# ml4ai/mliis

Hardware: AMD Instinct MI355X
Metric: inner-loop images/sec (EfficientLab-6-3, 224x224, 5-shot) (higher is better)
Workload: dtype f32 (the long-K decoder convs and their filter gradients with every operand split exactly into three bf16 terms on the matrix cores, 6 term products, f32 accumulate: fp32-equivalent products; everything else the fp32 instruction)

## Files before the change

### mliis_amd/csrc/dwmarch.hip

```cpp
#include "bn_fold.hpp"
#include "common.hpp"

namespace mliis {

constexpr int kDwmStoreAux = 2;
typedef unsigned dwm_u32x4 __attribute__((ext_vector_type(4)));
constexpr unsigned kDwmOob = 0xFFFFFFF0u;

__device__ __forceinline__ __amdgpu_buffer_rsrc_t dwm_rsrc(const void* p) {
  const unsigned long long u = (unsigned long long)p;
  const unsigned lo = __builtin_amdgcn_readfirstlane((unsigned)u), hi = __builtin_amdgcn_readfirstlane((unsigned)(u >> 32));
  return __builtin_amdgcn_make_buffer_rsrc((void*)(((unsigned long long)hi << 32) | lo), 0, 0x80000000u, 0x00020000);
}

typedef unsigned dwm_u32x2 __attribute__((ext_vector_type(2)));
template <typename T = float>
__device__ __forceinline__ float4 dwm_load(__amdgpu_buffer_rsrc_t r, int off, bool ok) {
  if constexpr (sizeof(T) == 4) {
    const dwm_u32x4 u = __builtin_amdgcn_raw_buffer_load_b128(r, ok ? off : (int)kDwmOob, 0, 0);
    return make_float4(__uint_as_float(u.x), __uint_as_float(u.y), __uint_as_float(u.z), __uint_as_float(u.w));
  } else {
    const dwm_u32x2 u = __builtin_amdgcn_raw_buffer_load_b64(r, ok ? off : (int)kDwmOob, 0, 0);
    return unpack_bf16x4(make_uint2(u.x, u.y));
  }
}

template <typename T = float>
__device__ __forceinline__ void dwm_store(__amdgpu_buffer_rsrc_t r, int off, bool ok, const float4 v) {
  if constexpr (sizeof(T) == 2) {
    const uint2 pk = pack_bf16x4(v);
    dwm_u32x2 u2;
    u2.x = pk.x; u2.y = pk.y;
    __builtin_amdgcn_raw_buffer_store_b64(u2, r, ok ? off : (int)kDwmOob, 0, kDwmStoreAux);
    return;
  }
  dwm_u32x4 u;
  u.x = __float_as_uint(v.x); u.y = __float_as_uint(v.y); u.z = __float_as_uint(v.z); u.w = __float_as_uint(v.w);
  __builtin_amdgcn_raw_buffer_store_b128(u, r, ok ? off : (int)kDwmOob, 0, kDwmStoreAux);
}
__device__ __forceinline__ float4 f4sel(bool ok, const float4 v) { return ok ? v : make_float4(0.f, 0.f, 0.f, 0.f); }
template <typename T> __device__ __forceinline__ float4 dwm_stored(const float4 v) { return stored_value(static_cast<const T*>(nullptr), v); }

template <int K, int S>
struct MarchCfg {
  static constexpr int TS = S == 1 ? 4 : 2;
  static constexpr int BW = 7 * TS;
  static constexpr int SPR = BW / TS;
  static constexpr int RS = 4;
  static constexpr int IBW = (BW - 1) * S + K;
  static constexpr int IBWP = (IBW + 1) & ~1;
  static constexpr int WIN = (RS - 1) * S + K;
  static constexpr int NEW = RS * S;
  static constexpr int NR = WIN + NEW;
  static constexpr int WW = (TS - 1) * S + K;
  static_assert(IBW <= 32, "one pixel lane per ring column");
  static_assert(WIN <= 2 * NEW, "head batch + batch 0 cover the window of step 0");
};

struct DwmBn {
  BnFold f;
  const float* gamma;
  const float* beta;
};

struct DwmDyBn {
  const float* z;
  const float *mean, *rstd, *gamma, *beta;
  const float *gate, *chan_add;
  const float* stage1;
  int nimg;
  double inv_rows;
  float *dgamma, *dbeta;
};
struct DwmDyQuad {
  float4 sc, sh, gt, ca, k1, k0;
};
__device__ __forceinline__ DwmDyQuad dwm_dybn_setup(const DwmDyBn& d, int C, int c0, int q, bool cok, int n, bool lead) {
  const int c = cok ? c0 + q * 4 : 0;
  const float4 m = ld4(d.mean + c), rs = ld4(d.rstd + c), ga = ld4(d.gamma + c), be = ld4(d.beta + c);
  DwmDyQuad k;
  k.gt = ld4(d.gate + (long long)n * C + c);
  k.ca = ld4(d.chan_add + (long long)n * C + c);
  double s1[4] = {0, 0, 0, 0}, s2[4] = {0, 0, 0, 0};
  for (int i0 = 0; i0 < d.nimg; i0 += 8) {
    float4 u[8], v[8];
#pragma unroll
    for (int j = 0; j < 8; ++j) {
      const int i = i0 + j < d.nimg ? i0 + j : d.nimg - 1;
      u[j] = ld4(d.stage1 + ((long long)i * 2 + 0) * C + c);
      v[j] = ld4(d.stage1 + ((long long)i * 2 + 1) * C + c);
    }
#pragma unroll
    for (int j = 0; j < 8; ++j)
      if (i0 + j < d.nimg) {
        s1[0] += u[j].x; s1[1] += u[j].y; s1[2] += u[j].z; s1[3] += u[j].w;
        s2[0] += v[j].x; s2[1] += v[j].y; s2[2] += v[j].z; s2[3] += v[j].w;
      }
  }
  if (lead && cok && (threadIdx.x >> 3) == 0) {
    st4(d.dbeta + c, make_float4((float)s1[0], (float)s1[1], (float)s1[2], (float)s1[3]));
    st4(d.dgamma + c, make_float4((float)s2[0], (float)s2[1], (float)s2[2], (float)s2[3]));
  }
  const float4 a = make_float4((float)(s1[0] * d.inv_rows), (float)(s1[1] * d.inv_rows), (float)(s1[2] * d.inv_rows), (float)(s1[3] * d.inv_rows));
  const float4 b = make_float4((float)(s2[0] * d.inv_rows), (float)(s2[1] * d.inv_rows), (float)(s2[2] * d.inv_rows), (float)(s2[3] * d.inv_rows));
  k.sc = f4mul(ga, rs);
  k.sh = make_float4(fmaf(-m.x, k.sc.x, be.x), fmaf(-m.y, k.sc.y, be.y), fmaf(-m.z, k.sc.z, be.z), fmaf(-m.w, k.sc.w, be.w));
  k.k1 = make_float4(-k.sc.x * b.x * rs.x, -k.sc.y * b.y * rs.y, -k.sc.z * b.z * rs.z, -k.sc.w * b.w * rs.w);
  k.k0 = make_float4(-k.sc.x * a.x - k.k1.x * m.x, -k.sc.y * a.y - k.k1.y * m.y, -k.sc.z * a.z - k.k1.z * m.z, -k.sc.w * a.w - k.k1.w * m.w);
  return k;
}
__device__ __forceinline__ float dwm_dz1(float da2, float z, float sc, float sh, float gt, float ca, float k1, float k0) {
  const float u = fmaf(z, sc, sh);
  const float sg = sigmoid_f(u);
  const float g = fmaf(da2, gt, ca) * (sg * (1.0f + u * (1.0f - sg)));
  return fmaf(sc, g, fmaf(z, k1, k0));
}
__device__ __forceinline__ float4 dwm_dz1(const float4 da2, const float4 z, const DwmDyQuad& k) {
  return make_float4(dwm_dz1(da2.x, z.x, k.sc.x, k.sh.x, k.gt.x, k.ca.x, k.k1.x, k.k0.x), dwm_dz1(da2.y, z.y, k.sc.y, k.sh.y, k.gt.y, k.ca.y, k.k1.y, k.k0.y),
                     dwm_dz1(da2.z, z.z, k.sc.z, k.sh.z, k.gt.z, k.ca.z, k.k1.z, k.k0.z), dwm_dz1(da2.w, z.w, k.sc.w, k.sh.w, k.gt.w, k.ca.w, k.k1.w, k.k0.w));
}

template <int NEW, bool TWO>
struct DwmBatch {
  float4 a[NEW];
  float4 b[TWO ? NEW : 1];
};

struct DwmArgs {
  const float* x;
  const float* w;
  float* y;
  int Hi, Wi, Ho, Wo;
  int C, pt, pl;
  int bands, bw, chunks, rpc;
  float* stats_part;
  DwmBn bn;
  DwmDyBn dyb;
  const float* z;
  float* dw_part;
};

struct DwmQuad {
  float4 sc, sh, m, rs;
};

__device__ __forceinline__ float4 dwm_act(const float4 z, const DwmQuad& k) {
  float4 u = make_float4(fmaf(z.x, k.sc.x, k.sh.x), fmaf(z.y, k.sc.y, k.sh.y), fmaf(z.z, k.sc.z, k.sh.z), fmaf(z.w, k.sc.w, k.sh.w));
  return make_float4(swish_f(u.x), swish_f(u.y), swish_f(u.z), swish_f(u.w));
}

constexpr int kDwmFoldBatch = 8;
template <bool FOLD>
struct DwmBnState {
  float4 g, b, m, rs;
  FoldAcc acc;
  float4 u[FOLD ? kDwmFoldBatch : 1], v[FOLD ? kDwmFoldBatch : 1];
  int k;
};
template <bool FOLD>
__device__ __forceinline__ void dwm_bn_begin(const DwmBn& bn, int C, int c0, int q, bool cok, DwmBnState<FOLD>& st) {
  const int c = cok ? c0 + q * 4 : 0;
  st.g = ld4(bn.gamma + c);
  st.b = ld4(bn.beta + c);
  if (FOLD && bn.f.nblk > 0) {
    const int bl = threadIdx.x >> 3;
    st.k = bl;
    for (; st.k + 32 * kDwmFoldBatch < bn.f.nblk; st.k += 32 * kDwmFoldBatch) {
      fold_issue<FOLD ? kDwmFoldBatch : 1>(bn.f.part, bn.f.nblk, C, c, st.k, bl, st.u, st.v);
      if (cok) fold_add<FOLD ? kDwmFoldBatch : 1>(st.acc, bn.f.nblk, st.k, st.u, st.v);
    }
    fold_issue<FOLD ? kDwmFoldBatch : 1>(bn.f.part, bn.f.nblk, C, c, st.k, st.k < bn.f.nblk ? st.k : 0, st.u, st.v);
  } else {
    st.m = ld4(bn.f.mean + c);
    st.rs = ld4(bn.f.rstd + c);
  }
}
template <bool FOLD>
__device__ __forceinline__ DwmQuad dwm_bn_end(const DwmBn& bn, int C, int c0, int q, bool cok, bool lead, double* smd, float* s_mr ,
                                              DwmBnState<FOLD>& st) {
  const int t = threadIdx.x;
  DwmQuad k;
  if (FOLD && bn.f.nblk > 0) {
    if (cok) fold_add<FOLD ? kDwmFoldBatch : 1>(st.acc, bn.f.nblk, st.k, st.u, st.v);
    double s, ss;
    fold_finish(st.acc, smd, s, ss);
    if (t < 32) {
      const double m = s * bn.f.inv_n;
      double var = ss * bn.f.inv_n - m * m;
      if (var < 0.0) var = 0.0;
      const float mf = (float)m, rf = (float)(1.0 / sqrt(var + (double)bn.f.eps));
      s_mr[t] = mf;
      s_mr[32 + t] = rf;
      const int cc = c0 + t;
      if (lead && cc < C) {
        bn.f.mean[cc] = mf;
        bn.f.rstd[cc] = rf;
        if (bn.f.moving_mean != nullptr) {
          const float mm = bn.f.moving_mean[cc], mv = bn.f.moving_var[cc];
          bn.f.moving_mean[cc] = mm - (mm - mf) * bn.f.one_minus_momentum;
          bn.f.moving_var[cc] = mv - (mv - (float)(var * (double)bn.f.ema_var_factor)) * bn.f.one_minus_momentum;
        }
      }
    }
    __syncthreads();
    k.m = ld4(s_mr + q * 4);
    k.rs = ld4(s_mr + 32 + q * 4);
    __syncthreads();
  } else {
    k.m = st.m;
    k.rs = st.rs;
  }
  k.sc = f4mul(st.g, k.rs);
  k.sh = make_float4(fmaf(-k.m.x, k.sc.x, st.b.x), fmaf(-k.m.y, k.sc.y, st.b.y), fmaf(-k.m.z, k.sc.z, st.b.z), fmaf(-k.m.w, k.sc.w, st.b.w));
  return k;
}

__device__ __forceinline__ void dwm_emit_pair(const float4 s1, const float4 s2, float4* buf, float* __restrict__ part, unsigned blk, int C,
                                              int c0) {
  const int t = threadIdx.x;
  buf[t] = s1;
  buf[256 + t] = s2;
  __syncthreads();
  float4 v = f4zero();
  if (t < 64) {
    const int qq = t & 7, g = (t >> 3) & 3, vv = t >> 5;
#pragma unroll
    for (int i = 0; i < 8; ++i) v = f4add(v, buf[vv * 256 + (g * 8 + i) * 8 + qq]);
  }
  __syncthreads();
  if (t < 64) buf[t] = v;
  __syncthreads();
  if (t < 16) {
    const int qq = t & 7, vv = t >> 3;
    const int cc = c0 + qq * 4;
    const float4* b4 = buf + vv * 32 + qq;
    if (cc < C) st4(part + ((long long)blk * 2 + vv) * C + cc, f4add(f4add(b4[0], b4[8]), f4add(b4[16], b4[24])));
  }
}

template <int K, int S, bool PRE, bool BWD, bool DYBN = false, typename TA = float, typename TB = float>
__global__ __launch_bounds__(256, BWD ? 1 : 2) void dwm_conv_k(const DwmArgs a) {
  constexpr int EA = (int)sizeof(TA), EB = (int)sizeof(TB);
  static_assert(!DYBN || BWD, "DYBN is a backward mode");
  typedef MarchCfg<K, S> G;
  constexpr int TS = G::TS, SPR = G::SPR, RS = G::RS, IBW = G::IBW, IBWP = G::IBWP, WIN = G::WIN, NEW = G::NEW, NR = G::NR, WW = G::WW;
  static_assert(!BWD || S == 1, "the stride-2 backward is dwm_bwd_s2_k");
  constexpr int kRingF4 = (NR * IBWP + 1) * 8;
  constexpr int kTrash = NR * IBWP * 8;
  constexpr int kScratchF4 = BWD ? (K * K * 4 * 8) : 0;
  constexpr int kSharedF4 = kRingF4 > kScratchF4 ? kRingF4 : kScratchF4;
  static_assert(kSharedF4 * 16 >= 2 * 32 * 32 * 8, "the statistics fold borrows the ring");
  __shared__ float4 ring[kSharedF4];
  __shared__ float4 wl[K * K * 8];
  __shared__ __attribute__((aligned(16))) float s_mr[64];

  const int t = threadIdx.x, q = t & 7, p = t >> 3;
  const unsigned bx = xcd_remap(blockIdx.x, gridDim.x);
  const int chunk = (int)(bx % (unsigned)a.chunks);
  const unsigned r_ = bx / (unsigned)a.chunks;
  const int band = (int)(r_ % (unsigned)a.bands), n = (int)(r_ / (unsigned)a.bands);
  const int c0 = blockIdx.y * 32, c = c0 + q * 4;
  const bool cok = c < a.C;
  const int Hi = a.Hi, Wi = a.Wi, Ho = a.Ho, Wo = a.Wo, C = a.C;
  const int oy0 = chunk * a.rpc;
  const int oy1 = oy0 + a.rpc < Ho ? oy0 + a.rpc : Ho;
  const int ox0 = band * a.bw;
  const int bwa = a.bw < Wo - ox0 ? a.bw : Wo - ox0;
  const int iy0 = oy0 * S - a.pt, ix0 = ox0 * S - a.pl;
  const int ibw = (bwa - 1) * S + K;
  const int rows_needed = (oy1 - oy0 - 1) * S + K;
  const int nsteps = (oy1 - oy0 + RS - 1) / RS;
  const __amdgpu_buffer_rsrc_t rX = dwm_rsrc(a.x);
  const __amdgpu_buffer_rsrc_t rZ = dwm_rsrc((BWD ? a.z : a.x));
  const __amdgpu_buffer_rsrc_t rY = dwm_rsrc(a.y);

  const bool colok = cok && p < ibw && (unsigned)(ix0 + p) < (unsigned)Wi;
  const int tbase = (((n * Hi + iy0) * Wi + ix0 + p) * C + c) * EA;
  const int rowbytes = Wi * C * EA;
  const int lcol = p < IBWP ? (p ^ ((p >> 2) & 1)) * 8 + q : kTrash + q;
  auto row_in = [&](int rr) { return rr >= 0 && rr < rows_needed && (unsigned)(iy0 + rr) < (unsigned)Hi; };
  typedef DwmBatch<NEW, DYBN> Batch;
  const __amdgpu_buffer_rsrc_t rX2 = dwm_rsrc(DYBN ? a.dyb.z : a.x);
  auto issue = [&](Batch& r, int rb) {
#pragma unroll
    for (int j = 0; j < NEW; ++j) {
      r.a[j] = dwm_load<TA>(rX, tbase + (rb + j) * rowbytes, colok && row_in(rb + j));
      if (DYBN) r.b[j] = dwm_load<TA>(rX2, tbase + (rb + j) * rowbytes, colok && row_in(rb + j));
    }
  };
  DwmQuad kq;
  DwmDyQuad dq;
  auto commit = [&](const Batch& r, int rb, int sb) {
#pragma unroll
    for (int j = 0; j < NEW; ++j) {
      float4 v = r.a[j];
      if (PRE && !BWD) v = f4sel(colok && row_in(rb + j), dwm_act(v, kq));
      if (DYBN) v = f4sel(colok && row_in(rb + j), dwm_dz1(v, r.b[j], dq));
      int slot = sb + j;
      if (slot >= NR) slot -= NR;
      if (rb + j >= 0) ring[(p < IBWP ? slot * (IBWP * 8) : 0) + lcol] = v;
    }
  };

  const int ro = p >> 3, sx = p & 7;
  const bool item_ok = sx < SPR && cok;
  const int colbase = sx < SPR ? sx * (TS * S) : 0;
  const int sxpar = sx & 1;
  const int zbase = BWD ? (((n * Ho + oy0 + ro) * Wo + ox0 + sx * TS) * C + c) * EB : 0;
  auto issue_z = [&](float4 (&zr)[TS], int step) {
    if (BWD) {
      const int oy = oy0 + step * RS + ro;
      const int base = zbase + step * RS * Wo * C * EB;
#pragma unroll
      for (int u = 0; u < TS; ++u) zr[u] = dwm_load<TB>(rZ, base + u * C * EB, item_ok && oy < oy1 && sx * TS + u < bwa);
    }
  };

  constexpr int HEAD = WIN - 2 * NEW;
  float4 wreg = f4zero();
  if (t < K * K * 8) {
    const int tap = t >> 3, qq = t & 7;
    const int cc = c0 + qq * 4;
    if (cc < C) wreg = ld4(a.w + (long long)(BWD ? K * K - 1 - tap : tap) * C + cc);
  }
  DwmBnState<!BWD> bst;
  if (PRE) dwm_bn_begin(a.bn, C, c0, q, cok, bst);
  if (DYBN) dq = dwm_dybn_setup(a.dyb, C, c0, q, cok, n, bx == 0);
  Batch ra, rb_;
  float4 za[TS], zb[TS];
  {
    Batch h0, h1;
    issue(h0, HEAD);
    issue(h1, WIN - NEW);
    issue_z(za, 0);
    if (PRE) kq = dwm_bn_end(a.bn, C, c0, q, cok, bx == 0, reinterpret_cast<double*>(ring), s_mr, bst);
    issue(ra, WIN);
    issue(rb_, WIN + NEW);
    issue_z(zb, 1);
    if (t < K * K * 8) wl[t] = wreg;
    commit(h0, HEAD, HEAD < 0 ? HEAD + NR : HEAD);
    commit(h1, WIN - NEW, (WIN - NEW) % NR);
  }
  __syncthreads();

  float4 s1 = f4zero(), s2 = f4zero();
  float4 dwacc[BWD ? K * K : 1];
  if (BWD) {
#pragma unroll
    for (int k = 0; k < K * K; ++k) dwacc[k] = f4zero();
  }

  int sw = 0;
  auto compute = [&](int step, const float4 (&zr)[TS]) {
    const int oy = oy0 + step * RS + ro;
    const bool row_ok = item_ok && oy < oy1;
    int s0 = sw + ro * S;
    if (s0 >= NR) s0 -= NR;
    float4 acc[TS];
#pragma unroll
    for (int u = 0; u < TS; ++u) acc[u] = f4zero();
    int wofs = q;
    if (K == 5) asm volatile("" : "+v"(wofs));
    const float4* wq = wl + wofs;
    float4 av[TS], sgm[TS];
    if (BWD) {
#pragma unroll
      for (int u = 0; u < TS; ++u) {
        const bool ok = row_ok && sx * TS + u < bwa;
        if (PRE) {
          const float4 z = zr[u];
          const float4 uu = make_float4(fmaf(z.x, kq.sc.x, kq.sh.x), fmaf(z.y, kq.sc.y, kq.sh.y), fmaf(z.z, kq.sc.z, kq.sh.z), fmaf(z.w, kq.sc.w, kq.sh.w));
          sgm[u] = f4sel(ok, make_float4(sigmoid_f(uu.x), sigmoid_f(uu.y), sigmoid_f(uu.z), sigmoid_f(uu.w)));
          av[u] = f4mul(uu, sgm[u]);
        } else {
          av[u] = f4sel(ok, zr[u]);
        }
      }
    }
    auto read_row = [&](int ky, float4 (&in)[WW]) {
      int slot = s0 + ky;
      if (slot >= NR) slot -= NR;
      if constexpr ((TS * S) % 4 == 0) {
        const float4* rowp = ring + slot * (IBWP * 8) + colbase * 8 + q;
        const float4* A0 = rowp + sxpar * 8;
        const float4* A1 = rowp - sxpar * 8;
#pragma unroll
        for (int j = 0; j < WW; ++j) {
          const int je = j ^ ((j >> 2) & 1);
          in[j] = ((je & 1) ? A1 : A0)[je * 8];
        }
      } else {
        const float4* rowp = ring + slot * (IBWP * 8) + q;
#pragma unroll
        for (int j = 0; j < WW; ++j) {
          const int col = colbase + j;
          in[j] = rowp[(col ^ ((col >> 2) & 1)) * 8];
        }
      }
    };
    auto fma_row = [&](int ky, const float4 (&in)[WW]) {
      float4 wk[K];
#pragma unroll
      for (int kx = 0; kx < K; ++kx) wk[kx] = wq[(ky * K + kx) * 8];
#pragma unroll
      for (int kx = 0; kx < K; ++kx)
#pragma unroll
        for (int u = 0; u < TS; ++u) {
          acc[u] = f4fma(in[u * S + kx], wk[kx], acc[u]);
          if (BWD) dwacc[ky * K + kx] = f4fma(in[u + kx], av[u], dwacc[ky * K + kx]);
        }
    };
    if (K == 3) {
      float4 in[WW];
#pragma unroll
      for (int ky = 0; ky < K; ++ky) {
        read_row(ky, in);
        fma_row(ky, in);
      }
    } else {
      float4 inA[WW], inB[WW];
      read_row(0, inA);
#pragma unroll
      for (int ky = 0; ky < K; ++ky) {
        if (ky + 1 < K) read_row(ky + 1, (ky & 1) ? inA : inB);
        fma_row(ky, (ky & 1) ? inB : inA);
        __builtin_amdgcn_sched_barrier(0);
      }
    }
    const int ybase = (((n * Ho + oy) * Wo + ox0 + sx * TS) * C + c) * EB;
    if (K == 5 && EB == 2) __builtin_amdgcn_sched_barrier(0);
#pragma unroll
    for (int u = 0; u < TS; ++u) {
      const bool ok = row_ok && sx * TS + u < bwa;
      if (!(K == 5 && !BWD)) acc[u] = dwm_stored<TB>(acc[u]);
      dwm_store<TB>(rY, ybase + u * C * EB, ok, acc[u]);
      if (!BWD) {
        const float4 v = f4sel(ok, acc[u]);
        s1 = f4add(s1, v);
        s2 = f4fma(v, v, s2);
      } else if (PRE) {
        const float4 z = zr[u], sg_ = sgm[u];
        const float4 uu = make_float4(fmaf(z.x, kq.sc.x, kq.sh.x), fmaf(z.y, kq.sc.y, kq.sh.y), fmaf(z.z, kq.sc.z, kq.sh.z), fmaf(z.w, kq.sc.w, kq.sh.w));
        const float4 g = make_float4(acc[u].x * sg_.x * (1.0f + uu.x * (1.0f - sg_.x)), acc[u].y * sg_.y * (1.0f + uu.y * (1.0f - sg_.y)),
                                     acc[u].z * sg_.z * (1.0f + uu.z * (1.0f - sg_.z)), acc[u].w * sg_.w * (1.0f + uu.w * (1.0f - sg_.w)));
        const float4 xh = make_float4((z.x - kq.m.x) * kq.rs.x, (z.y - kq.m.y) * kq.rs.y, (z.z - kq.m.z) * kq.rs.z, (z.w - kq.m.w) * kq.rs.w);
        s1 = f4add(s1, g);
        s2 = f4fma(g, xh, s2);
      }
    }
  };

  int rbn = WIN;
  int sbn = WIN % NR;
  for (int i = 0; i < nsteps; i += 2) {
    compute(i, za);
    commit(ra, rbn, sbn);
    issue(ra, rbn + 2 * NEW);
    issue_z(za, i + 2);
    rbn += NEW; sbn += NEW; if (sbn >= NR) sbn -= NR;
    sw += NEW; if (sw >= NR) sw -= NR;
    __syncthreads();
    if (i + 1 < nsteps) compute(i + 1, zb);
    commit(rb_, rbn, sbn);
    issue(rb_, rbn + 2 * NEW);
    issue_z(zb, i + 3);
    rbn += NEW; sbn += NEW; if (sbn >= NR) sbn -= NR;
    sw += NEW; if (sw >= NR) sw -= NR;
    __syncthreads();
  }

  if (a.stats_part != nullptr && (!BWD || PRE)) dwm_emit_pair(s1, s2, ring, a.stats_part, bx, C, c0);
  if (BWD) {
    __syncthreads();
    float4* fold = ring;
#pragma unroll
    for (int k = 0; k < K * K; ++k) {
      float4 v = dwacc[k];
#pragma unroll
      for (int off = 8; off < 64; off <<= 1) {
        v.x += __shfl_xor(v.x, off); v.y += __shfl_xor(v.y, off); v.z += __shfl_xor(v.z, off); v.w += __shfl_xor(v.w, off);
      }
      if ((t & 63) < 8) fold[(k * 4 + (t >> 6)) * 8 + q] = v;
    }
    __syncthreads();
    for (int e = t; e < K * K * 8; e += 256) {
      const int k = e >> 3, qq = e & 7;
      const int cc = c0 + qq * 4;
      if (cc < C)
        st4(a.dw_part + ((long long)bx * (K * K) + (K * K - 1 - k)) * C + cc,
            f4add(f4add(fold[(k * 4 + 0) * 8 + qq], fold[(k * 4 + 1) * 8 + qq]), f4add(fold[(k * 4 + 2) * 8 + qq], fold[(k * 4 + 3) * 8 + qq])));
    }
  }
}

template <int K, bool PRE, bool DYBN = false, typename TA = float, typename TB = float>
__global__ __launch_bounds__(256, (K == 5 || DYBN) ? 1 : 2) void dwm_bwd_s2_k(const DwmArgs a) {
  constexpr int EA = (int)sizeof(TA), EB = (int)sizeof(TB);
  constexpr int BP = 14;
  constexpr int D = (K - 1) / 2;
  constexpr int NEWD = 2, WIND = 2 + D, NR = WIND + NEWD, IBW = 16;
  static_assert(BP + D <= IBW, "one pixel lane per ring pixel of a batch");
  constexpr int kRingF4 = NR * IBW * 8;
  constexpr int kScratchF4 = K * K * 4 * 8;
  constexpr int kSharedF4 = (kRingF4 > kScratchF4 ? kRingF4 : kScratchF4) > 1024 ? (kRingF4 > kScratchF4 ? kRingF4 : kScratchF4) : 1024;
  __shared__ float4 ring[kSharedF4];
  __shared__ float4 wl[K * K * 8];
  __shared__ __attribute__((aligned(16))) float s_mr[64];

  const int t = threadIdx.x, q = t & 7, p = t >> 3;
  const unsigned bx = xcd_remap(blockIdx.x, gridDim.x);
  const int chunk = (int)(bx % (unsigned)a.chunks);
  const unsigned r_ = bx / (unsigned)a.chunks;
  const int band = (int)(r_ % (unsigned)a.bands), n = (int)(r_ / (unsigned)a.bands);
  const int c0 = blockIdx.y * 32, c = c0 + q * 4;
  const bool cok = c < a.C;
  const int Hd = a.Hi, Wd = a.Wi, H = a.Ho, W = a.Wo, C = a.C, pt = a.pt, pl = a.pl;
  const int my_lo = pt >> 1, my_hi = (H + pt - 1) >> 1;
  const int mx_lo = pl >> 1, mx_hi = (W + pl - 1) >> 1;
  const int m0 = my_lo + chunk * a.rpc;
  const int m1 = m0 + a.rpc <= my_hi + 1 ? m0 + a.rpc : my_hi + 1;
  const int x0 = mx_lo + band * a.bw;
  const int bpa = a.bw < mx_hi + 1 - x0 ? a.bw : mx_hi + 1 - x0;
  const int nsteps = (m1 - m0 + 1) / 2;
  const int rows_needed = m1 - m0 + D;
  const __amdgpu_buffer_rsrc_t rX = dwm_rsrc(a.x);
  const __amdgpu_buffer_rsrc_t rZ = dwm_rsrc(a.z);
  const __amdgpu_buffer_rsrc_t rY = dwm_rsrc(a.y);

  const int sl = p >> 4, scol = p & 15;
  const bool colok = cok && scol < bpa + D && (unsigned)(x0 - D + scol) < (unsigned)Wd;
  const int tbase = (((n * Hd + m0 - D + sl) * Wd + x0 - D + scol) * C + c) * EA;
  const int rowbytes = Wd * C * EA;
  typedef DwmBatch<1, DYBN> Batch;
  const __amdgpu_buffer_rsrc_t rX2 = dwm_rsrc(DYBN ? a.dyb.z : a.x);
  auto row_in = [&](int rr) { return rr >= 0 && rr < rows_needed && (unsigned)(m0 - D + rr) < (unsigned)Hd; };
  auto issue = [&](Batch& r, int rb) {
    r.a[0] = dwm_load<TA>(rX, tbase + rb * rowbytes, colok && row_in(rb + sl));
    if (DYBN) r.b[0] = dwm_load<TA>(rX2, tbase + rb * rowbytes, colok && row_in(rb + sl));
  };
  DwmDyQuad dq;
  auto commit = [&](const Batch& r, int rb, int sb) {
    int slot = sb + sl;
    if (slot >= NR) slot -= NR;
    float4 v = r.a[0];
    if (DYBN) v = f4sel(colok && row_in(rb + sl), dwm_dz1(v, r.b[0], dq));
    if (rb + sl >= 0) ring[slot * (IBW * 8) + scol * 8 + q] = v;
  };

  const int rp = p >> 4, px = p & 15;
  const bool item_ok = px < bpa && cok;
  const int pxc = px < BP ? px : 0;
  const int wi0 = 2 * (x0 + px) - pl;
  auto pix_ok = [&](int step, int u) {
    const int hi = 2 * (m0 + 2 * step + rp) + (u >> 1) - pt, wi = wi0 + (u & 1);
    return item_ok && m0 + 2 * step + rp < m1 && (unsigned)hi < (unsigned)H && (unsigned)wi < (unsigned)W;
  };
  auto pix_off = [&](int step, int u) {
    const int hi = 2 * (m0 + 2 * step + rp) + (u >> 1) - pt, wi = wi0 + (u & 1);
    return (((n * H + hi) * W + wi) * C + c) * EB;
  };
  auto issue_z = [&](float4 (&zr)[4], int step) {
#pragma unroll
    for (int u = 0; u < 4; ++u) zr[u] = dwm_load<TB>(rZ, pix_off(step, u), pix_ok(step, u));
  };

  constexpr int HEAD = WIND - 2 * NEWD;
  float4 wreg = f4zero();
  if (t < K * K * 8) {
    const int tap = t >> 3, qq = t & 7;
    const int cc = c0 + qq * 4;
    if (cc < C) wreg = ld4(a.w + (long long)tap * C + cc);
  }
  DwmQuad kq;
  DwmBnState<false> bst;
  if (PRE) dwm_bn_begin(a.bn, C, c0, q, cok, bst);
  if (PRE) kq = dwm_bn_end(a.bn, C, c0, q, cok, false, reinterpret_cast<double*>(ring), s_mr, bst);
  if (DYBN) dq = dwm_dybn_setup(a.dyb, C, c0, q, cok, n, bx == 0);
  Batch ra, rb_, h0, h1;
  float4 za[4], zb[4];
  issue(h0, HEAD);
  issue(h1, WIND - NEWD);
  issue_z(za, 0);
  issue(ra, WIND);
  issue(rb_, WIND + NEWD);
  issue_z(zb, 1);
  if (t < K * K * 8) wl[t] = wreg;
  commit(h0, HEAD, HEAD < 0 ? HEAD + NR : HEAD);
  commit(h1, WIND - NEWD, (WIND - NEWD) % NR);
  __syncthreads();

  float4 s1 = f4zero(), s2 = f4zero();
  float4 dwacc[K * K];
#pragma unroll
  for (int k = 0; k < K * K; ++k) dwacc[k] = f4zero();

  int sw = 0;
  auto compute = [&](int step, const float4 (&zr)[4]) {
    float4 av[4], sgm[4], acc[4];
#pragma unroll
    for (int u = 0; u < 4; ++u) {
      const bool ok = pix_ok(step, u);
      acc[u] = f4zero();
      if (PRE) {
        const float4 z = zr[u];
        const float4 uu = make_float4(fmaf(z.x, kq.sc.x, kq.sh.x), fmaf(z.y, kq.sc.y, kq.sh.y), fmaf(z.z, kq.sc.z, kq.sh.z), fmaf(z.w, kq.sc.w, kq.sh.w));
        sgm[u] = f4sel(ok, make_float4(sigmoid_f(uu.x), sigmoid_f(uu.y), sigmoid_f(uu.z), sigmoid_f(uu.w)));
        av[u] = f4mul(uu, sgm[u]);
      } else {
        av[u] = f4sel(ok, zr[u]);
      }
    }
    int s0 = sw + rp;
    if (s0 >= NR) s0 -= NR;
    int wofs = q;
    if (K == 5) asm volatile("" : "+v"(wofs));
    const float4* wq = wl + wofs;
#pragma unroll
    for (int wr = 0; wr <= D; ++wr) {
      int slot = s0 + wr;
      if (slot >= NR) slot -= NR;
      const float4* rowp = ring + slot * (IBW * 8) + pxc * 8 + q;
      float4 dv[D + 1];
#pragma unroll
      for (int wc = 0; wc <= D; ++wc) dv[wc] = rowp[wc * 8];
#pragma unroll
      for (int pa = 0; pa < 2; ++pa) {
        const int ky = pa + 2 * (D - wr);
        if (ky > K - 1) continue;
#pragma unroll
        for (int wc = 0; wc <= D; ++wc)
#pragma unroll
          for (int pb = 0; pb < 2; ++pb) {
            const int kx = pb + 2 * (D - wc);
            if (kx > K - 1) continue;
            const int u = pa * 2 + pb, tap = ky * K + kx;
            acc[u] = f4fma(dv[wc], wq[tap * 8], acc[u]);
            dwacc[tap] = f4fma(dv[wc], av[u], dwacc[tap]);
          }
      }
      __builtin_amdgcn_sched_barrier(0);
    }
#pragma unroll
    for (int u = 0; u < 4; ++u) {
      acc[u] = dwm_stored<TB>(acc[u]);
      dwm_store<TB>(rY, pix_off(step, u), pix_ok(step, u), acc[u]);
      if (PRE) {
        const float4 z = zr[u], sg_ = sgm[u];
        const float4 uu = make_float4(fmaf(z.x, kq.sc.x, kq.sh.x), fmaf(z.y, kq.sc.y, kq.sh.y), fmaf(z.z, kq.sc.z, kq.sh.z), fmaf(z.w, kq.sc.w, kq.sh.w));
        const float4 g = make_float4(acc[u].x * sg_.x * (1.0f + uu.x * (1.0f - sg_.x)), acc[u].y * sg_.y * (1.0f + uu.y * (1.0f - sg_.y)),
                                     acc[u].z * sg_.z * (1.0f + uu.z * (1.0f - sg_.z)), acc[u].w * sg_.w * (1.0f + uu.w * (1.0f - sg_.w)));
        const float4 xh = make_float4((z.x - kq.m.x) * kq.rs.x, (z.y - kq.m.y) * kq.rs.y, (z.z - kq.m.z) * kq.rs.z, (z.w - kq.m.w) * kq.rs.w);
        s1 = f4add(s1, g);
        s2 = f4fma(g, xh, s2);
      }
    }
  };

  int rbn = WIND, sbn = WIND % NR;
  for (int i = 0; i < nsteps; i += 2) {
    compute(i, za);
    commit(ra, rbn, sbn);
    issue(ra, rbn + 2 * NEWD);
    issue_z(za, i + 2);
    rbn += NEWD; sbn += NEWD; if (sbn >= NR) sbn -= NR;
    sw += NEWD; if (sw >= NR) sw -= NR;
    __syncthreads();
    if (i + 1 < nsteps) compute(i + 1, zb);
    commit(rb_, rbn, sbn);
    issue(rb_, rbn + 2 * NEWD);
    issue_z(zb, i + 3);
    rbn += NEWD; sbn += NEWD; if (sbn >= NR) sbn -= NR;
    sw += NEWD; if (sw >= NR) sw -= NR;
    __syncthreads();
  }

  if (a.stats_part != nullptr && PRE) dwm_emit_pair(s1, s2, ring, a.stats_part, bx, C, c0);
  __syncthreads();
  float4* fold = ring;
#pragma unroll
  for (int k = 0; k < K * K; ++k) {
    float4 v = dwacc[k];
#pragma unroll
    for (int off = 8; off < 64; off <<= 1) {
      v.x += __shfl_xor(v.x, off); v.y += __shfl_xor(v.y, off); v.z += __shfl_xor(v.z, off); v.w += __shfl_xor(v.w, off);
    }
    if ((t & 63) < 8) fold[(k * 4 + (t >> 6)) * 8 + q] = v;
  }
  __syncthreads();
  for (int e = t; e < K * K * 8; e += 256) {
    const int k = e >> 3, qq = e & 7;
    const int cc = c0 + qq * 4;
    if (cc < C)
      st4(a.dw_part + ((long long)bx * (K * K) + k) * C + cc,
          f4add(f4add(fold[(k * 4 + 0) * 8 + qq], fold[(k * 4 + 1) * 8 + qq]), f4add(fold[(k * 4 + 2) * 8 + qq], fold[(k * 4 + 3) * 8 + qq])));
  }
}

struct MarchGeom {
  int bands, bw, chunks, rpc;
  int Ho, Wo, pt, pl;
  long long gx;
  int gy;
};

static inline void same_pad(int H, int K, int S, int* Ho, int* pt) {
  *Ho = (H + S - 1) / S;
  int th = (*Ho - 1) * S + K - H;
  if (th < 0) th = 0;
  *pt = th / 2;
}

static int g_dwm_target = -1;
static inline int dwm_target(bool bwd) {
  if (g_dwm_target < 0) {
    const char* e = getenv("MLIIS_DWM_TARGET");
    g_dwm_target = e ? atoi(e) : 0;
    if (g_dwm_target < 0) g_dwm_target = 0;
  }
  return g_dwm_target ? g_dwm_target : (bwd ? 256 : 448);
}

static inline void march_split(int N, int cgs, int P, int Q, int unit, int bmax, int ts, bool bwd, MarchGeom* g) {
  g->bands = (Q + bmax - 1) / bmax;
  int bw = (Q + g->bands - 1) / g->bands;
  bw = (bw + ts - 1) / ts * ts;
  g->bw = bw;
  g->bands = (Q + bw - 1) / bw;
  const long long base = (long long)N * cgs * g->bands;
  long long chunks = dwm_target(bwd) / base;
  const int max_chunks = (P + 2 * unit - 1) / (2 * unit);
  if (chunks > max_chunks) chunks = max_chunks;
  if (chunks < 1) chunks = 1;
  int rpc = (int)((P + chunks - 1) / chunks);
  rpc = (rpc + unit - 1) / unit * unit;
  g->rpc = rpc;
  g->chunks = (P + rpc - 1) / rpc;
  g->gx = (long long)N * g->bands * g->chunks;
  g->gy = cgs;
}

static inline MarchGeom march_geom_fwd(int N, int H, int W, int C, int K, int S) {
  MarchGeom g;
  same_pad(H, K, S, &g.Ho, &g.pt);
  same_pad(W, K, S, &g.Wo, &g.pl);
  if (S == 1) march_split(N, ceil_div(C, 32), g.Ho, g.Wo, 4, 28, 4, false, &g);
  else march_split(N, ceil_div(C, 32), g.Ho, g.Wo, 4, 14, 2, false, &g);
  return g;
}

static inline MarchGeom march_geom_bwd(int N, int H, int W, int C, int K, int S) {
  MarchGeom g;
  same_pad(H, K, S, &g.Ho, &g.pt);
  same_pad(W, K, S, &g.Wo, &g.pl);
  if (S == 1) {
    march_split(N, ceil_div(C, 32), H, W, 4, 28, 4, true, &g);
  } else {
    const int py = ((H + g.pt - 1) >> 1) - (g.pt >> 1) + 1, pxn = ((W + g.pl - 1) >> 1) - (g.pl >> 1) + 1;
    march_split(N, ceil_div(C, 32), py, pxn, 2, 14, 1, true, &g);
  }
  return g;
}

static inline DwmBn make_bn(const float* part, int nblk, long long count, const float* gamma, const float* beta, float* mean, float* rstd,
                            float* moving_mean, float* moving_var, float eps, float momentum, int unbiased) {
  DwmBn b;
  b.f.part = part;
  b.f.nblk = nblk;
  b.f.inv_n = 1.0 / (double)count;
  b.f.eps = eps;
  b.f.one_minus_momentum = 1.0f - momentum;
  b.f.ema_var_factor = (unbiased && count > 1) ? (float)((double)count / (double)(count - 1)) : 1.0f;
  b.f.mean = mean;
  b.f.rstd = rstd;
  b.f.moving_mean = moving_mean;
  b.f.moving_var = moving_var;
  b.gamma = gamma;
  b.beta = beta;
  return b;
}

static inline bool dwm_types_ok(bool bwd, int ta, int tb) {
  if (ta == MLIIS_DT_F32 && tb == MLIIS_DT_F32) return true;
  if (ta == MLIIS_DT_BF16 && tb == MLIIS_DT_BF16) return true;
  return bwd ? (ta == MLIIS_DT_BF16 && tb == MLIIS_DT_F32) : (ta == MLIIS_DT_F32 && tb == MLIIS_DT_BF16);
}
template <int K, int S, bool PRE, bool BWD>
static void launch_conv(const MarchGeom& g, const DwmArgs& a, int ta, int tb, hipStream_t stream) {
  const dim3 grid((unsigned)g.gx, g.gy);
  if (ta == MLIIS_DT_F32 && tb == MLIIS_DT_F32) hipLaunchKernelGGL((dwm_conv_k<K, S, PRE, BWD, false, float, float>), grid, dim3(256), 0, stream, a);
  else if (ta == MLIIS_DT_BF16 && tb == MLIIS_DT_BF16) hipLaunchKernelGGL((dwm_conv_k<K, S, PRE, BWD, false, bf16s, bf16s>), grid, dim3(256), 0, stream, a);
  else if constexpr (BWD) hipLaunchKernelGGL((dwm_conv_k<K, S, PRE, BWD, false, bf16s, float>), grid, dim3(256), 0, stream, a);
  else hipLaunchKernelGGL((dwm_conv_k<K, S, PRE, BWD, false, float, bf16s>), grid, dim3(256), 0, stream, a);
}
template <int K, bool PRE>
static void launch_bwd_s2(const MarchGeom& g, const DwmArgs& a, int ta, int tb, hipStream_t stream) {
  const dim3 grid((unsigned)g.gx, g.gy);
  if (ta == MLIIS_DT_F32) hipLaunchKernelGGL((dwm_bwd_s2_k<K, PRE, false, float, float>), grid, dim3(256), 0, stream, a);
  else if (tb == MLIIS_DT_BF16) hipLaunchKernelGGL((dwm_bwd_s2_k<K, PRE, false, bf16s, bf16s>), grid, dim3(256), 0, stream, a);
  else hipLaunchKernelGGL((dwm_bwd_s2_k<K, PRE, false, bf16s, float>), grid, dim3(256), 0, stream, a);
}
template <int K, typename TA, typename TB>
static void launch_bwd_dybn_t(const MarchGeom& g, const DwmArgs& a, int stride, hipStream_t stream) {
  const dim3 grid((unsigned)g.gx, g.gy);
  if (stride == 1) hipLaunchKernelGGL((dwm_conv_k<K, 1, true, true, true, TA, TB>), grid, dim3(256), 0, stream, a);
  else hipLaunchKernelGGL((dwm_bwd_s2_k<K, true, true, TA, TB>), grid, dim3(256), 0, stream, a);
}
template <int K>
static void launch_bwd_dybn(const MarchGeom& g, const DwmArgs& a, int stride, int ta, int tb, hipStream_t stream) {
  if (ta == MLIIS_DT_F32) launch_bwd_dybn_t<K, float, float>(g, a, stride, stream);
  else if (tb == MLIIS_DT_BF16) launch_bwd_dybn_t<K, bf16s, bf16s>(g, a, stride, stream);
  else launch_bwd_dybn_t<K, bf16s, float>(g, a, stride, stream);
}

}

using namespace mliis;

static int dwm_check(const char* name, int N, int H, int W, int C, int k, int stride) {
  MLIIS_REQUIRE(N > 0 && H > 0 && W > 0 && C > 0 && (C & 3) == 0, MLIIS_ERR_ARG, "%s: bad shape N=%d H=%d W=%d C=%d (C %% 4 must be 0)", name, N, H,
                W, C);
  MLIIS_REQUIRE((k == 3 || k == 5) && (stride == 1 || stride == 2), MLIIS_ERR_UNSUPPORTED, "%s: unsupported k=%d stride=%d", name, k, stride);
  MLIIS_REQUIRE((long long)N * H * W * C * 4 < (1LL << 31), MLIIS_ERR_UNSUPPORTED, "%s: tensor larger than 2 GiB (32-bit buffer offsets)", name);
  return MLIIS_OK;
}

extern "C" {

int mliis_dwconv_bn_supported(int N, int H, int W, int C, int k, int stride) {
  if (N <= 0 || H <= 0 || W <= 0 || C <= 0 || (C & 3) || (k != 3 && k != 5) || (stride != 1 && stride != 2)) return 0;
  return ((long long)N * H * W * C * 4 < (1LL << 31)) ? 1 : 0;
}

int mliis_dwconv_bn_fwd_blocks(int N, int H, int W, int C, int k, int stride) {
  if (N <= 0 || H <= 0 || W <= 0 || C <= 0 || (C & 3) || (k != 3 && k != 5) || (stride != 1 && stride != 2)) return 0;
  return (int)march_geom_fwd(N, H, W, C, k, stride).gx;
}

int mliis_dwconv_bn_bwd_blocks(int N, int H, int W, int C, int k, int stride) {
  if (N <= 0 || H <= 0 || W <= 0 || C <= 0 || (C & 3) || (k != 3 && k != 5) || (stride != 1 && stride != 2)) return 0;
  return (int)march_geom_bwd(N, H, W, C, k, stride).gx;
}

int mliis_dwconv_bn_fwd(const float* z, const float* bn_part, int bn_nblk, const float* bn_gamma, const float* bn_beta, float* bn_mean,
                        float* bn_rstd, float* bn_moving_mean, float* bn_moving_var, float eps, float momentum, const float* w, float* y,
                        int N, int H, int W, int C, int k, int stride, float* stats_part, size_t stats_floats, int* stats_nblk,
                        int in_dtype, int out_dtype, hipStream_t stream) {
  int rc = dwm_check("dwconv_bn_fwd", N, H, W, C, k, stride);
  if (rc) return rc;
  MLIIS_REQUIRE(dwm_types_ok(false, in_dtype, out_dtype), MLIIS_ERR_ARG, "dwconv_bn_fwd: unsupported storage types (in %d, out %d)", in_dtype, out_dtype);
  MLIIS_REQUIRE(z && w && y && aligned16(z) && aligned16(w) && aligned16(y), MLIIS_ERR_ARG, "dwconv_bn_fwd: null or unaligned pointer");
  const bool pre = bn_gamma != nullptr;
  if (pre) {
    MLIIS_REQUIRE(bn_beta && bn_mean && bn_rstd && aligned16(bn_gamma) && aligned16(bn_beta), MLIIS_ERR_ARG,
                  "dwconv_bn_fwd: the batch norm needs gamma, beta (16-byte aligned) and mean / rstd vectors");
    MLIIS_REQUIRE(bn_nblk >= 0 && (bn_nblk == 0 || (bn_part && aligned16(bn_part))), MLIIS_ERR_ARG, "dwconv_bn_fwd: bad statistics partials");
    MLIIS_REQUIRE((bn_moving_mean == nullptr) == (bn_moving_var == nullptr), MLIIS_ERR_ARG, "dwconv_bn_fwd: moving mean / variance come as a pair");
  }
  const MarchGeom g = march_geom_fwd(N, H, W, C, k, stride);
  MLIIS_REQUIRE(g.gx < (1LL << 31), MLIIS_ERR_UNSUPPORTED, "dwconv_bn_fwd: too many workgroups");
  if (stats_nblk) *stats_nblk = 0;
  if (stats_part != nullptr) {
    MLIIS_REQUIRE(stats_nblk && aligned16(stats_part), MLIIS_ERR_ARG, "dwconv_bn_fwd: statistics need a 16-byte aligned buffer and a stats_nblk output");
    MLIIS_REQUIRE((size_t)g.gx * 2 * C <= stats_floats, MLIIS_ERR_WORKSPACE, "dwconv_bn_fwd: statistics buffer too small (%zu floats needed, %zu given)",
                  (size_t)g.gx * 2 * C, stats_floats);
    *stats_nblk = (int)g.gx;
  }
  DwmArgs a{};
  a.x = z; a.w = w; a.y = y;
  a.Hi = H; a.Wi = W; a.Ho = g.Ho; a.Wo = g.Wo; a.C = C; a.pt = g.pt; a.pl = g.pl;
  a.bands = g.bands; a.bw = g.bw; a.chunks = g.chunks; a.rpc = g.rpc;
  a.stats_part = stats_part;
  if (pre) a.bn = make_bn(bn_part, bn_nblk, (long long)N * H * W, bn_gamma, bn_beta, bn_mean, bn_rstd, bn_moving_mean, bn_moving_var, eps, momentum, 0);
#define DWM_FWD(K_, S_)                                             \
  do {                                                              \
    if (pre) launch_conv<K_, S_, true, false>(g, a, in_dtype, out_dtype, stream);  \
    else launch_conv<K_, S_, false, false>(g, a, in_dtype, out_dtype, stream);     \
  } while (0)
  if (k == 3 && stride == 1) DWM_FWD(3, 1);
  else if (k == 3) DWM_FWD(3, 2);
  else if (stride == 1) DWM_FWD(5, 1);
  else DWM_FWD(5, 2);
#undef DWM_FWD
  MLIIS_CHECK_LAUNCH("dwconv_bn_fwd");
  return MLIIS_OK;
}

int mliis_dwconv_bn_bwd(const float* dy, const float* z, const float* bn_mean, const float* bn_rstd, const float* bn_gamma,
                        const float* bn_beta, const float* w, float* dx, float* dw, int N, int H, int W, int C, int k, int stride,
                        float* dw_part, size_t dw_part_floats, float* bn_part, size_t bn_part_floats, int* nblk, int dy_dtype, int zx_dtype,
                        hipStream_t stream) {
  int rc = dwm_check("dwconv_bn_bwd", N, H, W, C, k, stride);
  if (rc) return rc;
  MLIIS_REQUIRE(dwm_types_ok(true, dy_dtype, zx_dtype), MLIIS_ERR_ARG, "dwconv_bn_bwd: unsupported storage types (dy %d, z / dx %d)", dy_dtype, zx_dtype);
  MLIIS_REQUIRE(dy && z && w && dx && dw_part && nblk && aligned16(dy) && aligned16(z) && aligned16(w) && aligned16(dx) && aligned16(dw_part),
                MLIIS_ERR_ARG, "dwconv_bn_bwd: null or unaligned pointer");
  const bool pre = bn_gamma != nullptr;
  if (pre)
    MLIIS_REQUIRE(bn_beta && bn_mean && bn_rstd && aligned16(bn_gamma) && aligned16(bn_beta) && (bn_part == nullptr || aligned16(bn_part)),
                  MLIIS_ERR_ARG, "dwconv_bn_bwd: the batch norm needs gamma, beta (16-byte aligned), mean and rstd");
  const MarchGeom g = march_geom_bwd(N, H, W, C, k, stride);
  MLIIS_REQUIRE(g.gx < (1LL << 31), MLIIS_ERR_UNSUPPORTED, "dwconv_bn_bwd: too many workgroups");
  MLIIS_REQUIRE((size_t)g.gx * k * k * C <= dw_part_floats, MLIIS_ERR_WORKSPACE, "dwconv_bn_bwd: filter-gradient slabs need %zu floats, %zu given",
                (size_t)g.gx * k * k * C, dw_part_floats);
  MLIIS_REQUIRE(!pre || bn_part == nullptr || (size_t)g.gx * 2 * C <= bn_part_floats, MLIIS_ERR_WORKSPACE,
                "dwconv_bn_bwd: batch-norm partials need %zu floats, %zu given", (size_t)g.gx * 2 * C, bn_part_floats);
  *nblk = (int)g.gx;
  DwmArgs a{};
  a.x = dy; a.w = w; a.y = dx; a.z = z;
  a.C = C;
  a.bands = g.bands; a.bw = g.bw; a.chunks = g.chunks; a.rpc = g.rpc;
  a.stats_part = pre ? bn_part : nullptr;
  a.dw_part = dw_part;
  if (pre) a.bn = make_bn(nullptr, 0, 1, bn_gamma, bn_beta, const_cast<float*>(bn_mean), const_cast<float*>(bn_rstd), nullptr, nullptr, 0.f, 0.f, 0);
  if (stride == 1) {
    a.Hi = H; a.Wi = W; a.Ho = H; a.Wo = W; a.pt = k - 1 - g.pt; a.pl = k - 1 - g.pl;
    if (k == 3) { if (pre) launch_conv<3, 1, true, true>(g, a, dy_dtype, zx_dtype, stream); else launch_conv<3, 1, false, true>(g, a, dy_dtype, zx_dtype, stream); }
    else { if (pre) launch_conv<5, 1, true, true>(g, a, dy_dtype, zx_dtype, stream); else launch_conv<5, 1, false, true>(g, a, dy_dtype, zx_dtype, stream); }
  } else {
    a.Hi = g.Ho; a.Wi = g.Wo; a.Ho = H; a.Wo = W; a.pt = g.pt; a.pl = g.pl;
    if (k == 3) { if (pre) launch_bwd_s2<3, true>(g, a, dy_dtype, zx_dtype, stream); else launch_bwd_s2<3, false>(g, a, dy_dtype, zx_dtype, stream); }
    else { if (pre) launch_bwd_s2<5, true>(g, a, dy_dtype, zx_dtype, stream); else launch_bwd_s2<5, false>(g, a, dy_dtype, zx_dtype, stream); }
  }
  MLIIS_CHECK_LAUNCH("dwconv_bn_bwd");
  if (dw != nullptr) {
    MLIIS_REQUIRE(aligned16(dw), MLIIS_ERR_ALIGN, "dwconv_bn_bwd: dw must be 16-byte aligned");
    hipLaunchKernelGGL(fold_flat_k, dim3(ceil_div(k * k * C, kFoldX)), dim3(kFoldX, kFoldY), 0, stream, dw_part, (int)g.gx, (long long)k * k * C, 1.0f,
                       dw, 0, (long long)k * k * C, 0LL, 0LL);
    MLIIS_CHECK_LAUNCH("dwconv_bn_bwd_fold");
  }
  return MLIIS_OK;
}

int mliis_mbconv_dw_bwd_march(const float* da2, const float* z1, const float* mean1, const float* rstd1, const float* gamma1, const float* beta1,
                              const float* gate, const float* chan_add, const float* stage1, int stage1_nimg, float* dgamma1, float* dbeta1,
                              const float* z0, const float* mean0, const float* rstd0, const float* gamma0, const float* beta0, const float* w,
                              float* dx, int N, int H, int W, int C, int k, int stride, float* dw_part, size_t dw_part_floats, float* bn_part,
                              size_t bn_part_floats, int* nblk, int dy_dtype, int zx_dtype, hipStream_t stream) {
  int rc = dwm_check("mbconv_dw_bwd_march", N, H, W, C, k, stride);
  if (rc) return rc;
  MLIIS_REQUIRE(dwm_types_ok(true, dy_dtype, zx_dtype), MLIIS_ERR_ARG, "mbconv_dw_bwd_march: unsupported storage types (da2 / z1 %d, z0 / dx %d)", dy_dtype, zx_dtype);
  MLIIS_REQUIRE(da2 && z1 && mean1 && rstd1 && gamma1 && beta1 && gate && chan_add && stage1 && stage1_nimg > 0 && dgamma1 && dbeta1 && z0 && mean0 &&
                    rstd0 && gamma0 && beta0 && w && dx && dw_part && bn_part && nblk,
                MLIIS_ERR_ARG, "mbconv_dw_bwd_march: null pointer");
  MLIIS_REQUIRE(aligned16(da2) && aligned16(z1) && aligned16(mean1) && aligned16(rstd1) && aligned16(gamma1) && aligned16(beta1) && aligned16(gate) &&
                    aligned16(chan_add) && aligned16(stage1) && aligned16(dgamma1) && aligned16(dbeta1) && aligned16(z0) && aligned16(mean0) &&
                    aligned16(rstd0) && aligned16(gamma0) && aligned16(beta0) && aligned16(w) && aligned16(dx) && aligned16(dw_part) && aligned16(bn_part),
                MLIIS_ERR_ALIGN, "mbconv_dw_bwd_march: pointers must be 16-byte aligned");
  const MarchGeom g = march_geom_bwd(N, H, W, C, k, stride);
  MLIIS_REQUIRE(g.gx < (1LL << 31), MLIIS_ERR_UNSUPPORTED, "mbconv_dw_bwd_march: too many workgroups");
  MLIIS_REQUIRE((size_t)g.gx * k * k * C <= dw_part_floats && (size_t)g.gx * 2 * C <= bn_part_floats, MLIIS_ERR_WORKSPACE,
                "mbconv_dw_bwd_march: slab buffers too small (%zu / %zu floats needed)", (size_t)g.gx * k * k * C, (size_t)g.gx * 2 * C);
  *nblk = (int)g.gx;
  DwmArgs a{};
  a.x = da2; a.w = w; a.y = dx; a.z = z0;
  a.C = C;
  a.bands = g.bands; a.bw = g.bw; a.chunks = g.chunks; a.rpc = g.rpc;
  a.stats_part = bn_part;
  a.dw_part = dw_part;
  a.bn = make_bn(nullptr, 0, 1, gamma0, beta0, const_cast<float*>(mean0), const_cast<float*>(rstd0), nullptr, nullptr, 0.f, 0.f, 0);
  a.dyb = DwmDyBn{z1, mean1, rstd1, gamma1, beta1, gate, chan_add, stage1, stage1_nimg, 1.0 / ((double)N * g.Ho * g.Wo), dgamma1, dbeta1};
  if (stride == 1) {
    a.Hi = H; a.Wi = W; a.Ho = H; a.Wo = W; a.pt = k - 1 - g.pt; a.pl = k - 1 - g.pl;
  } else {
    a.Hi = g.Ho; a.Wi = g.Wo; a.Ho = H; a.Wo = W; a.pt = g.pt; a.pl = g.pl;
  }
  if (k == 3) launch_bwd_dybn<3>(g, a, stride, dy_dtype, zx_dtype, stream);
  else launch_bwd_dybn<5>(g, a, stride, dy_dtype, zx_dtype, stream);
  MLIIS_CHECK_LAUNCH("mbconv_dw_bwd_march");
  return MLIIS_OK;
}
}
```

Before: 3669.

## Fold 5x5 depthwise filter-gradient rows through LDS per kernel row

For the K=5 backward depthwise kernel, each thread now keeps 5 per-row filter-gradient partials instead of 25 register accumulators. After each kernel row it reduces them across lane pairs with DPP and across wave row-groups through a small per-wave LDS stage, accumulating only into its own kx slot. This cuts register pressure in the register-heavy backward kernel and shortens the final shuffle reduction. The cost is extra LDS traffic, wave barriers and DPP adds on every kernel row.

Measured after the change: 3674 (median of 6 runs). No clear change (+0.1%).

```diff
diff --git a/mliis_amd/csrc/dwmarch.hip b/mliis_amd/csrc/dwmarch.hip
--- a/mliis_amd/csrc/dwmarch.hip
+++ b/mliis_amd/csrc/dwmarch.hip
@@ -238,6 +238,58 @@
   }
 }
 
+constexpr int kDwmRowStageF4 = 4 * 5 * 8;
+__device__ __forceinline__ float dwm_single(float v) {
+  asm("" : "+v"(v));
+  return v;
+}
+__device__ __forceinline__ float dwm_pair_add(float v) {
+  v = dwm_single(v);
+  return dwm_single(v + __builtin_bit_cast(float, __builtin_amdgcn_update_dpp(0, __builtin_bit_cast(int, v), 0x128, 0xF, 0xF, true)));
+}
+__device__ __forceinline__ void dwm_wave_lds_order() {
+  __builtin_amdgcn_fence(__ATOMIC_RELEASE, "wavefront");
+  __builtin_amdgcn_wave_barrier();
+  __builtin_amdgcn_fence(__ATOMIC_ACQUIRE, "wavefront");
+}
+typedef float dwm_f32x2 __attribute__((ext_vector_type(2)));
+__device__ __forceinline__ void dwm_pin(float4& v) {
+  dwm_f32x2 lo = {v.x, v.y}, hi = {v.z, v.w};
+  asm volatile("" : "+v"(lo), "+v"(hi));
+  v = make_float4(lo.x, lo.y, hi.x, hi.y);
+}
+struct DwmRowPend {
+  float4 p[4];
+};
+struct DwmRowFold {
+  float4* wr;
+  const float4* rd;
+  bool odd;
+  __device__ __forceinline__ void init(float4* stage) {
+    const int lane = threadIdx.x & 63, q = lane & 7, pl = lane >> 3;
+    float4* w = stage + (threadIdx.x >> 6) * kDwmRowStageF4;
+    odd = pl & 1;
+    wr = w + ((pl >> 1) * 5 + (odd ? 3 : 0)) * 8 + q;
+    rd = w + (pl < 5 ? pl : 4) * 8 + q;
+  }
+  static __device__ __forceinline__ float4 pair_add(const float4 v) {
+    return make_float4(dwm_pair_add(v.x), dwm_pair_add(v.y), dwm_pair_add(v.z), dwm_pair_add(v.w));
+  }
+  __device__ __forceinline__ void stage(const float4 (&r)[5], DwmRowPend& pend) const {
+    const float4 s0 = pair_add(r[0]), s1 = pair_add(r[1]), s2 = pair_add(r[2]), s3 = pair_add(r[3]), s4 = pair_add(r[4]);
+    dwm_wave_lds_order();
+    wr[0] = make_float4(odd ? s3.x : s0.x, odd ? s3.y : s0.y, odd ? s3.z : s0.z, odd ? s3.w : s0.w);
+    wr[8] = make_float4(odd ? s4.x : s1.x, odd ? s4.y : s1.y, odd ? s4.z : s1.z, odd ? s4.w : s1.w);
+    if (!odd) wr[16] = s2;
+    dwm_wave_lds_order();
+#pragma unroll
+    for (int j = 0; j < 4; ++j) pend.p[j] = rd[j * 5 * 8];
+  }
+  static __device__ __forceinline__ void finish(const DwmRowPend& pend, float4& total) {
+    total = f4add(total, f4add(f4add(pend.p[0], pend.p[1]), f4add(pend.p[2], pend.p[3])));
+  }
+};
+
 template <int K, int S, bool PRE, bool BWD, bool DYBN = false, typename TA = float, typename TB = float>
 __global__ __launch_bounds__(256, BWD ? 1 : 2) void dwm_conv_k(const DwmArgs a) {
   constexpr int EA = (int)sizeof(TA), EB = (int)sizeof(TB);
@@ -250,8 +302,10 @@
   constexpr int kScratchF4 = BWD ? (K * K * 4 * 8) : 0;
   constexpr int kSharedF4 = kRingF4 > kScratchF4 ? kRingF4 : kScratchF4;
   static_assert(kSharedF4 * 16 >= 2 * 32 * 32 * 8, "the statistics fold borrows the ring");
+  constexpr bool ROWS = BWD && K == 5;
   __shared__ float4 ring[kSharedF4];
   __shared__ float4 wl[K * K * 8];
+  __shared__ float4 dwstage[ROWS ? 4 * kDwmRowStageF4 : 1];
   __shared__ __attribute__((aligned(16))) float s_mr[64];
 
   const int t = threadIdx.x, q = t & 7, p = t >> 3;
@@ -344,11 +398,14 @@
   __syncthreads();
 
   float4 s1 = f4zero(), s2 = f4zero();
-  float4 dwacc[BWD ? K * K : 1];
+  constexpr int NDW = BWD ? (ROWS ? K : K * K) : 1;
+  float4 dwacc[NDW];
   if (BWD) {
 #pragma unroll
-    for (int k = 0; k < K * K; ++k) dwacc[k] = f4zero();
-  }
+    for (int k = 0; k < NDW; ++k) dwacc[k] = f4zero();
+  }
+  DwmRowFold rf;
+  if (ROWS) rf.init(dwstage);
 
   int sw = 0;
   auto compute = [&](int step, const float4 (&zr)[TS]) {
@@ -398,17 +455,36 @@
         }
       }
     };
+    DwmRowPend pend;
     auto fma_row = [&](int ky, const float4 (&in)[WW]) {
       float4 wk[K];
 #pragma unroll
       for (int kx = 0; kx < K; ++kx) wk[kx] = wq[(ky * K + kx) * 8];
-#pragma unroll
-      for (int kx = 0; kx < K; ++kx)
-#pragma unroll
-        for (int u = 0; u < TS; ++u) {
-          acc[u] = f4fma(in[u * S + kx], wk[kx], acc[u]);
-          if (BWD) dwacc[ky * K + kx] = f4fma(in[u + kx], av[u], dwacc[ky * K + kx]);
+      if constexpr (ROWS) {
+        float4 rw[5];
+#pragma unroll
+        for (int kx = 0; kx < K; ++kx) {
+          rw[kx] = f4zero();
+#pragma unroll
+          for (int u = 0; u < TS; ++u) {
+            acc[u] = f4fma(in[u * S + kx], wk[kx], acc[u]);
+            rw[kx] = f4fma(in[u + kx], av[u], rw[kx]);
+          }
         }
+#pragma unroll
+        for (int u = 0; u < TS; ++u) dwm_pin(acc[u]);
+        if (ky > 0) DwmRowFold::finish(pend, dwacc[ky > 0 ? ky - 1 : 0]);
+        rf.stage(rw, pend);
+        if (ky == K - 1) DwmRowFold::finish(pend, dwacc[K - 1]);
+      } else {
+#pragma unroll
+        for (int kx = 0; kx < K; ++kx)
+#pragma unroll
+          for (int u = 0; u < TS; ++u) {
+            acc[u] = f4fma(in[u * S + kx], wk[kx], acc[u]);
+            if (BWD) dwacc[ky * K + kx] = f4fma(in[u + kx], av[u], dwacc[ky * K + kx]);
+          }
+      }
     };
     if (K == 3) {
       float4 in[WW];
@@ -473,14 +549,21 @@
   if (BWD) {
     __syncthreads();
     float4* fold = ring;
-#pragma unroll
-    for (int k = 0; k < K * K; ++k) {
-      float4 v = dwacc[k];
-#pragma unroll
-      for (int off = 8; off < 64; off <<= 1) {
-        v.x += __shfl_xor(v.x, off); v.y += __shfl_xor(v.y, off); v.z += __shfl_xor(v.z, off); v.w += __shfl_xor(v.w, off);
-      }
-      if ((t & 63) < 8) fold[(k * 4 + (t >> 6)) * 8 + q] = v;
+    if constexpr (ROWS) {
+      if ((t & 63) < K * 8) {
+#pragma unroll
+        for (int ky = 0; ky < K; ++ky) fold[((ky * K + ((t & 63) >> 3)) * 4 + (t >> 6)) * 8 + q] = dwacc[ky];
+      }
+    } else {
+#pragma unroll
+      for (int k = 0; k < K * K; ++k) {
+        float4 v = dwacc[k];
+#pragma unroll
+        for (int off = 8; off < 64; off <<= 1) {
+          v.x += __shfl_xor(v.x, off); v.y += __shfl_xor(v.y, off); v.z += __shfl_xor(v.z, off); v.w += __shfl_xor(v.w, off);
+        }
+        if ((t & 63) < 8) fold[(k * 4 + (t >> 6)) * 8 + q] = v;
+      }
     }
     __syncthreads();
     for (int e = t; e < K * K * 8; e += 256) {
```
